# kaushikcfd/feinsum

Measured on AMD Instinct MI355X. Metric: GFLOP/s on DG-wave p=4 grad einsum (1e6 elems per GPU, fp64); fraction of roofline in `roofline`, higher is better.
Workload: dtype f64

## Files before the change

### feinsum_amd/_hip.py

```python

from __future__ import annotations

import ctypes as C
import os
from pathlib import Path
from typing import Optional, Sequence, Tuple

import numpy as np

from feinsum_amd.diagnostics import HipLibraryError, InvalidParameterError

FE_OK, FE_EINVAL, FE_EUNSUPPORTED, FE_EHIP = 0, -1, -2, -3
VARIANT_AUTO, VARIANT_GENERIC, VARIANT_MFMA, VARIANT_TILED, VARIANT_MFMA_SPLIT = 0, 1, 2, 3, 4
VARIANTS = {"auto": VARIANT_AUTO, "generic": VARIANT_GENERIC, "mfma": VARIANT_MFMA, "tiled": VARIANT_TILED,
            "mfma_split": VARIANT_MFMA_SPLIT}

FAMILY_F32 = 0x100
FAMILY_ACC = 0x200
FAMILY_FIELDS_F32 = 0x400


class ArgPack(C.Structure):

    _fields_ = [
# ... 79 lines not shown
    "fe_launch": (_int, [_i32, C.POINTER(ArgPack), _p]),
    "fe_grad3d_mixed_f64": (_int, [_p, _p, _pp, _pp, _i64, _i32, _i32, _i32, _p]),
    "fe_div3d_mixed_f64": (_int, [_p, _p, _pp, _pp, _i64, _i32, _i32, _i32, _p]),
    "fe_facemass_mixed_f64": (_int, [_p, _p, _pp, _pp, _i64, _i32, _i32, _i32, _i32, _i32, _p]),
    "fe_grad3d_strided_f64": (_int, [_p, _i64, _p, _pp, _pp, _i64, _i64, _i32, _i32, _i32, _p]),
    "fe_div3d_strided_f64": (_int, [_p, _i64, _p, _pp, _i64, _pp, _i64, _i32, _i32, _i32, _p]),
    "fe_facemass_strided_f64": (_int, [_p, _i64, _p, _pp, _i64, _pp, _i64, _i32, _i32, _i32, _i32, _i32, _p]),
    "fe_launch_f32": (_int, [_i32, C.POINTER(ArgPack), _p]),
    "fe_set_tail_rounds": (_int, [_i32]),
    "fe_set_tail_min_rounds": (_int, [_i32]),
    "fe_stream_retired": (_int, [_p]),
    "fe_tail_check": (_int, [_i32, C.POINTER(_i64), C.POINTER(_i32), C.POINTER(_i32), C.POINTER(_i32)]),
    "fe_capture_id": (_int, [_p, C.POINTER(C.c_uint64)]),
    "fe_graph_retired": (_int, [C.c_uint64]),
    "fe_tail_stats": (_int, [C.POINTER(_i64), _i32]),
    "fe_tail_plant": (_int, [_p, C.c_uint32]),
    "fe_set_temporal_loads_mib": (_int, [_i32]),
    "fe_set_write_through_mib": (_int, [_i32]),
    "fe_last_launch_info": (_int, [C.POINTER(_i64), _i32]),
    "fe_set_div_interleave": (_i64, [_i64]),
    "fe_set_div_quarter_tail": (_int, [_i32]),
    "fe_set_grad_quarter_tail": (_int, [_i32]),
    "fe_set_grad_staggered_start": (_int, [_i32]),
    "fe_set_phase_priority_p5": (_int, [_i32]),
    "fe_set_cu_limit": (_int, [_i32]),
    "fe_time_launches": (_int, [_i32, C.POINTER(ArgPack), _i32, _p, C.POINTER(C.c_float)]),
    "fe_einsum_generic": (_int, [C.POINTER(EinsumDesc), _pp, _p, _p]),
    "fe_einsum_contract": (_int, [C.POINTER(EinsumDesc), _pp, _p, _p]),
    "fe_einsum_contract_groups": (_int, [C.POINTER(EinsumDesc), C.POINTER(_i32), C.POINTER(_i32)]),
    "fe_einsum_reduce_plan": (_int, [C.POINTER(EinsumDesc), C.POINTER(_i32), C.POINTER(_i64), C.POINTER(_size)]),
    "fe_einsum_reduce": (_int, [C.POINTER(EinsumDesc), _pp, _p, _p, _size, _p]),
    "fe_geomadj_f64": (_int, [_p, _p, _p, _p, _i64, _i32, _i32, _i32, _i32, _i64, _i64, _i64, _p]),
    "fe_facemass_adj_f64": (_int, [_p, _p, _pp, _pp, _pp, _p, _i64, _i32, _i32, _i32, _i32, _i32, _p]),
    "fe_opgrad_plan": (_int, [_i64, _i32, C.POINTER(_i64), C.POINTER(_size)]),
    "fe_opgrad_f64": (_int, [_p, _pp, _pp, _p, _i64, _i32, _i32, _i32, _i32, _i64, _i64, _i64, _i64, _i64, _i64, _p, _size,
                          _p]),
    "fe_facemass_opgrad_f64": (_int, [_p, _pp, _pp, _p, _i64, _i32, _i32, _i32, _i32, _i32, _p, _size, _p]),
}
EXPORTED_SYMBOLS = tuple(SIGNATURES)


def library_path() -> Path:
    env = os.environ.get("FEINSUM_HIP_LIB")
    return Path(env) if env else Path(__file__).resolve().parent / "libfeinsum_hip.so"


# ... 432 lines not shown
    d["mixed_fields"] = bool(d["kind"] & 32)
    d["plain_field_loads"] = bool(d["kind"] & 64)
    d["element_slice"] = bool(d["kind"] & 128)
    d["kind"] = "B build interleaved" if d["kind"] & 4 else "default"
    return d


def set_phase_priority_p5(on: bool) -> bool:
    return bool(load_library().fe_set_phase_priority_p5(1 if on else 0))


def set_div_quarter_tail(on: bool) -> bool:
    return bool(load_library().fe_set_div_quarter_tail(1 if on else 0))


def set_grad_quarter_tail(on: bool) -> bool:
    return bool(load_library().fe_set_grad_quarter_tail(int(on)))


def set_grad_staggered_start(on: bool) -> bool:
    return bool(load_library().fe_set_grad_staggered_start(1 if on else 0))


def set_div_interleave(tiles: int) -> int:
    return int(load_library().fe_set_div_interleave(int(tiles)))


def set_write_through_mib(mib: int) -> int:
    return int(load_library().fe_set_write_through_mib(int(mib)))


def set_temporal_loads_mib(mib: int) -> int:
    return int(load_library().fe_set_temporal_loads_mib(int(mib)))
```

### feinsum_amd/csrc/fe_common.h

```cpp
#pragma once
#include <hip/hip_runtime.h>
#include <stdint.h>

namespace fe {

typedef double v4d __attribute__((ext_vector_type(4)));
typedef double v2d __attribute__((ext_vector_type(2)));

#define FE_AS1 __attribute__((address_space(1)))
#define FE_AS3 __attribute__((address_space(3)))

constexpr int kMaxFields = 8;
struct FieldPtrs {
    const double* v[kMaxFields];
    double* out[kMaxFields];
};

__device__ __forceinline__ const double* field_in(const FieldPtrs& P, int k) {
    const double* p = P.v[0];
#pragma unroll
    for (int q = 1; q < kMaxFields; ++q) p = (k == q) ? P.v[q] : p;
    return p;
}
__device__ __forceinline__ double* field_out(const FieldPtrs& P, int k) {
// ... 236 lines not shown

__device__ __forceinline__ void balance_priority(bool younger_half, int iteration) {
    if (younger_half) {
        if (iteration & 1) __builtin_amdgcn_s_setprio(1);
        else __builtin_amdgcn_s_setprio(0);
    }
}

template <class F>
__device__ __forceinline__ void remainder_items(int64_t e_begin, int64_t E, int Np, unsigned bid, unsigned nblk,
                                                F item) {
    const int64_t n = (E - e_begin) * Np;
    if (n <= 0) return;
    const unsigned per = blockDim.x;
    const int64_t want = (n + per - 1) / per;
    const unsigned k = want < (int64_t)nblk ? (unsigned)want : nblk;
    const unsigned half = (nblk + 1) / 2;
    const unsigned first = half >= k ? half - k : 0;
    if (bid < first || bid >= first + k) return;
    for (int64_t idx = (int64_t)(bid - first) * per + threadIdx.x; idx < n; idx += (int64_t)k * per)
        item(e_begin + idx / Np, (int)(idx % Np));
}

}
```

### feinsum_amd/csrc/fe_grad.h

```cpp
#pragma once
#include <type_traits>

#include "fe_common.h"
#include "fe_generic.h"

namespace fe {

constexpr int grad_row_tiles(int np) {
    int t = 1;
    while (4 * ((4 * t) / 3) < np) ++t;
    return t;
}

template <int NP, int M>
struct GradGeom {
    static constexpr int TEL = 16 * M;
    static constexpr int RT = grad_row_tiles(NP);
    static constexpr int TG = (4 * RT) / 3;
    static constexpr int KS = (NP + 3) / 4;
    static constexpr int TILE_D = TEL * NP;
    static constexpr int SUB_D = 16 * NP;
    static constexpr int U_CHUNKS = TILE_D / 2;
    static constexpr int U_INSTR = (U_CHUNKS + 63) / 64;
    static constexpr int J_ROW_CHUNKS = TEL / 2;
    static constexpr int J_CHUNKS = 9 * J_ROW_CHUNKS;
    static constexpr int J_INSTR = (J_CHUNKS + 63) / 64;
    static constexpr int SUB_CHUNKS = SUB_D / 2;
    static constexpr int SUB_INSTR = (SUB_CHUNKS + 63) / 64;
    static constexpr int LOADS = U_INSTR + J_INSTR;
    static constexpr int PLANE_STORES = M * SUB_INSTR;
    static constexpr int STORES = 3 * PLANE_STORES;
    static constexpr int ACC_LOADS = STORES;
    struct WaveLds {
        double u[2][TILE_D];
        double j[2][9 * TEL];
    };
    struct WaveOut {
        double o[2][SUB_D];
    };
    static constexpr int WAVES = 4;
    static constexpr int OP_D = 3 * NP * NP;
    static constexpr int IN_BYTES = (int)sizeof(WaveLds) * WAVES;
    static constexpr int OUT_BYTES = (int)sizeof(WaveOut) * WAVES;
    static constexpr int OP_BYTES = (OP_D * 8 + 15) / 16 * 16;
    static constexpr int LDS_BYTES = IN_BYTES + (OUT_BYTES > OP_BYTES ? OUT_BYTES : OP_BYTES);
    static_assert(4 * TG >= NP, "row permutation must cover every i");
    static_assert(LOADS + STORES + ACC_LOADS <= 60, "counted vmcnt must fit the 6-bit field");
    static_assert(2 * LDS_BYTES <= 160 * 1024, "two blocks per CU");
};

struct GradFields {
    const double* j[3];
    const double* u[kMaxFields];
    double* out[kMaxFields][3];
};

__device__ __forceinline__ const double* grad_field_u(const GradFields& P, int k) {
    const double* p = P.u[0];
#pragma unroll
    for (int q = 1; q < kMaxFields; ++q) p = (k == q) ? P.u[q] : p;
    return p;
}
__device__ __forceinline__ double* grad_plane_out(const GradFields& P, int k, int x) {
    double* p = P.out[0][x];
#pragma unroll
    for (int q = 1; q < kMaxFields; ++q) p = (k == q) ? P.out[q][x] : p;
    return p;
}
// ... 20 lines not shown
            J[(int64_t)(x * 3 + 2) * E + e] * t2;
}

__device__ __forceinline__ void grad3d_item_ld(const double* __restrict__ J, const double* __restrict__ D,
                                               const double* __restrict__ u, double* __restrict__ out, int64_t ldJ,
                                               int64_t ldOut, int Np, int64_t e, int i, int opT) {
    double t0 = 0.0, t1 = 0.0, t2 = 0.0;
    const double* ue = u + e * Np;
    const int si = opT ? 1 : Np, sj = opT ? Np : 1;
    const double* d0 = D + (int64_t)0 * Np * Np + (int64_t)i * si;
    const double* d1 = D + (int64_t)1 * Np * Np + (int64_t)i * si;
    const double* d2 = D + (int64_t)2 * Np * Np + (int64_t)i * si;
#pragma unroll 5
    for (int j = 0; j < Np; ++j) {
        const double uj = ue[j];
        t0 += d0[j * sj] * uj;
        t1 += d1[j * sj] * uj;
        t2 += d2[j * sj] * uj;
    }
    for (int x = 0; x < 3; ++x)
        out[((int64_t)x * ldOut + e) * Np + i] =
            J[(int64_t)(x * 3 + 0) * ldJ + e] * t0 + J[(int64_t)(x * 3 + 1) * ldJ + e] * t1 +
            J[(int64_t)(x * 3 + 2) * ldJ + e] * t2;
}

__global__ __launch_bounds__(256) void grad3d_generic_ld_kernel(
    const double* __restrict__ J, const double* __restrict__ D, const double* __restrict__ u,
    double* __restrict__ out, int64_t E, int64_t ldJ, int64_t ldOut, int Np, int opT) {
    const int64_t idx = (int64_t)blockIdx.x * 256 + threadIdx.x;
    if (idx >= E * Np) return;
    grad3d_item_ld(J, D, u, out, ldJ, ldOut, Np, idx / Np, (int)(idx % Np), opT);
}

__device__ __forceinline__ void grad3d_item_acc(const double* __restrict__ J, const double* __restrict__ D,
                                                const double* __restrict__ u, double* __restrict__ out, int64_t E,
                                                int Np, int64_t e, int i, int opT, double alpha, double beta) {
    double t0 = 0.0, t1 = 0.0, t2 = 0.0;
    const double* ue = u + e * Np;
    const int si = opT ? 1 : Np, sj = opT ? Np : 1;
    const double* d0 = D + (int64_t)0 * Np * Np + (int64_t)i * si;
    const double* d1 = D + (int64_t)1 * Np * Np + (int64_t)i * si;
    const double* d2 = D + (int64_t)2 * Np * Np + (int64_t)i * si;
#pragma unroll 5
    for (int j = 0; j < Np; ++j) {
        const double uj = ue[j];
        t0 += d0[j * sj] * uj;
// ... 88 lines not shown
            fe::fe_dbg_tile[GLOBAL_WAVE][LANE] = reinterpret_cast<unsigned long long*>(LDS_END)[(WAVE) * 16 + (LANE)];   \
    } while (0)
#else
#define FE_TILE_STAMP(ENABLED, LDS_END, WAVE, LANE, IT, K) do {} while (0)
#define FE_TILE_STAMPS_OUT(ENABLED, LDS_END, WAVE, LANE, GLOBAL_WAVE) do {} while (0)
#endif

template <int N>
struct GradOldValues {
    v2d v[2][N];
};
template <>
struct GradOldValues<0> {};
template <int NP, int N>
__device__ __forceinline__ void grad_load_old(const double* op, int lane, v2d (&dst)[N]) {
    constexpr int CHUNKS = 16 * NP / 2;
#pragma unroll
    for (int c = 0; c < N; ++c) {
        const int qc = c * 64 + lane;
        if ((c + 1) * 64 <= CHUNKS || qc < CHUNKS) dst[c] = __builtin_nontemporal_load(reinterpret_cast<const v2d*>(op + 2 * qc));
    }
}

template <int NP, int M, int kDbg = 0, bool kPlain = true, bool kPrep = false, bool kDyn = false, bool kAcc = false, bool kLd = false>
__device__ __forceinline__ void grad3d_mfma_body(
    const GradFields& P, const double* __restrict__ D, const void* __restrict__ prep, int nb, int nx_, int64_t E,
    int64_t nTiles, int op_flags, const unsigned bid, const unsigned nblk, unsigned* __restrict__ tail = nullptr,
    int64_t t_static = 0, const double alpha = 1.0, const double beta = 0.0, const int64_t ldJ = 0, const int64_t ldOut = 0) {
    static_assert(!kDyn || (kPlain && !kPrep), "dynamic walk: plain launches of one field");
    static_assert(!kLd || (kPlain && !kPrep && !kAcc && kDbg == 0), "element slices: plain grad, the plain operator");
    static_assert(!kAcc || (kPlain && !kPrep && !kDyn && kDbg == 0), "accumulating launches: plain grad, static walk, the plain operator");
    constexpr bool kAccAhead = kAcc && NP != 35;
    const bool acc_reads = kAcc && beta != 0.0;
    const int opT = op_flags & 1;
    const bool tload = (op_flags & kOpLoadsTemporal) != 0;
    const bool wthrough = kPlain && !kAcc && (op_flags & kOpStoresWriteThrough) != 0;
    const int nx = kPlain ? 3 : nx_;
    using G = GradGeom<NP, M>;
    using WaveLds = typename G::WaveLds;
    extern __shared__ __attribute__((aligned(16))) char smem[];
#ifdef FE_EXPERIMENTS
    const unsigned long long t_entry = (kDbg & 32) ? __builtin_amdgcn_s_memrealtime() : 0;
#endif
    if constexpr (kPlain && !kPrep && !kDyn && M == 1 && !kAcc && !kLd) {
        if ((op_flags & kOpStaggeredStart) && ((bid >> 3) & 1))
            for (int i = 0; i < kStaggerSleeps; ++i) __builtin_amdgcn_s_sleep(16);
    }
    const int lane = threadIdx.x & 63;
    const int wave = __builtin_amdgcn_readfirstlane(threadIdx.x >> 6);
    WaveLds* L = reinterpret_cast<WaveLds*>(smem) + wave;
    typename G::WaveOut* LO = reinterpret_cast<typename G::WaveOut*>(smem + G::IN_BYTES) + wave;
    const int n = lane & 15, g = lane >> 4;
#ifdef FE_EXPERIMENTS
    constexpr bool x_no_mfma = (kDbg & 1) != 0, x_no_stores = (kDbg & 2) != 0, x_plain_stores = (kDbg & 4) != 0, x_no_loads = (kDbg & 8) != 0,
// ... 37 lines not shown
        else grad_issue_j<NP, M, kPlain>(P, E, phys(tile), lane, lds_addr_uniform(L->j[0]));
        if (nb > 1) {
            grad_issue_u<NP, M, kNT>(P.u[1], phys(tile), lane, lds_addr_uniform(L->u[1]), tload);
            pre = true;
            return 1;
        }
        return 3;
    };
    auto remainder = [&](const double* Dsrc) {
        remainder_items(nTiles * G::TEL, E, NP, bid, nblk, [&](int64_t e, int i) {
            for (int k = 0; k < nb; ++k) {
                const double* uk = grad_field_u(P, k);
                if (kPlain) {
                    if constexpr (kLd) grad3d_item_ld(P.j[0], Dsrc, uk, grad_plane_out(P, k, 0), ldJ, ldOut, NP, e, i, opT);
                    else if constexpr (kAcc) grad3d_item_acc(P.j[0], Dsrc, uk, grad_plane_out(P, k, 0), E, NP, e, i, opT, alpha, beta);
                    else grad3d_item(P.j[0], Dsrc, uk, grad_plane_out(P, k, 0), E, NP, e, i, opT);
                } else {
                    double* const o[3] = {grad_plane_out(P, k, 0), grad_plane_out(P, k, 1), grad_plane_out(P, k, 2)};
#pragma unroll
                    for (int x = 0; x < 3; ++x)
                        if (o[x]) divcomp3d_item(P.j[x], Dsrc, uk, o[x], E, NP, e, i, opT, 0);
                }
            }
        });
    };
    int dbg_it = 0;
#ifdef FE_EXPERIMENTS
    if ((kDbg & 32) && lane < 16) reinterpret_cast<unsigned long long*>(smem + G::LDS_BYTES)[wave * 16 + lane] = 0;
#endif
    auto compute_unit = [&](int64_t tile_, int fk, const double* ut, const double* jt, auto with_acc) {
        constexpr bool kHaveAcc = decltype(with_acc)::value;
        FE_TILE_STAMP(x_stamps, smem + G::LDS_BYTES, wave, lane, dbg_it, 0);
        double* out_x[3];
        out_x[0] = grad_plane_out(P, fk, 0);
        if constexpr (kLd) out_x[1] = out_x[0] + ldOut * NP;
        else out_x[1] = kPlain ? out_x[0] + E * NP : grad_plane_out(P, fk, 1);
        if constexpr (kLd) out_x[2] = out_x[0] + 2 * ldOut * NP;
        else out_x[2] = kPlain ? out_x[0] + 2 * E * NP : grad_plane_out(P, fk, 2);
        int obuf = 0;
        const int64_t e0 = phys(tile_) * G::TEL;
        GradOldValues<kAcc ? G::SUB_INSTR : 0> old;
        if constexpr (kAccAhead) {
            if (acc_reads) grad_load_old<NP>(out_x[0] + e0 * NP, lane, old.v[0]);
        }
#pragma unroll
        for (int m = 0; m < M; ++m) {
// ... 258 lines not shown
        fk = nk;
        tile = nt;
        ub ^= 1;
        if (next_new_tile) jbuf ^= 1;
    };
    auto first_top = [&]() {
        if constexpr (kDyn) {
            if (use_dyn) {
                dyn_init();
                dyn_top();
                return;
            }
        }
        static_top();
    };

    if constexpr (kPrep) {
        load_prepared_fragments<G::RT * G::KS>(prep, lane, [&](int f, double v) { afrag[f / G::KS][f % G::KS] = v; });
        issue_first_units();
        prepared_fragments_landed();
        remainder(D);
    } else {
        stage_operator_dma<G::OP_D>(D, lds_addr_uniform(smem + G::IN_BYTES), wave, lane);
        const int units_issued = issue_first_units();
        switch (units_issued) {
            case 1: wait_vmcnt<G::LOADS + G::U_INSTR>(); break;
            case 3: wait_vmcnt<G::LOADS>(); break;
            default: wait_vmcnt<0>(); break;
        }
#ifdef FE_EXPERIMENTS
        if ((kDbg & 32) && lane == 0 && bid * G::WAVES + wave < 4096) fe_dbg_phase[bid * G::WAVES + wave][0] = __builtin_amdgcn_s_memrealtime();
#endif
        __syncthreads();
#ifdef FE_EXPERIMENTS
        if ((kDbg & 32) && lane == 0 && bid * G::WAVES + wave < 4096) fe_dbg_phase[bid * G::WAVES + wave][1] = __builtin_amdgcn_s_memrealtime();
#endif

        const double* dl = reinterpret_cast<const double*>(smem + G::IN_BYTES);
        remainder(dl);
        const int gp = n & 3, q = n >> 2;
        const int istride = opT ? 1 : NP, jstride = opT ? NP : 1;
        if constexpr (kFusedFirst) {
            static_assert(4 * (G::RT - 1) <= 3 * G::TG && 3 * G::TG + (4 * (G::RT - 1) - 1) / 3 < NP && 4 * G::KS - 5 < NP,
                          "padding rows in the last row tile only, padding columns in the last k-step only");
            const double* rowp[G::RT];
            bool rowok_last = true;
#pragma unroll
            for (int t = 0; t < G::RT; ++t) {
                const int s_ = 4 * t + q;
                const int r = s_ % 3, i = G::TG * gp + s_ / 3;
                if (t == G::RT - 1) rowok_last = (s_ < 3 * G::TG) && (i < NP);
                rowp[t] = dl + r * (NP * NP) + (i < NP ? i : 0) * istride + g * jstride;
            }
            const bool jok_last = 4 * (G::KS - 1) + g < NP;
            static_assert(4 * G::KS - NP <= 1 && (G::OP_D + NP + 1) * 8 <= G::LDS_BYTES - G::IN_BYTES, "the padding column stays inside the staging area");
            const int kstep = 4 * jstride;
            auto read_step = [&](int ks) {
#pragma unroll
                for (int t = 0; t < G::RT; ++t) afrag[t][ks] = rowp[t][ks * kstep];
            };
            auto fix_step = [&](int ks) {
#pragma unroll
// ... 147 lines not shown
            }
            wave_lds_fence();
        }
    }
    if constexpr (kDyn) {
        if (reportedb) {
            const unsigned pool_blocks = (nblk / (8 * kTailPools)) * 8 + (unsigned)max(0, min(8, (int)(nblk % (8 * kTailPools)) - 8 * pool));
            const unsigned before = tail_wait<G::STORES, 1>();
            if (before + 1 == pool_blocks * G::WAVES && lane == 0) {
                __hip_atomic_store(counter, 0u, __ATOMIC_RELAXED, __HIP_MEMORY_SCOPE_AGENT);
                __hip_atomic_store(done, 0u, __ATOMIC_RELAXED, __HIP_MEMORY_SCOPE_AGENT);
            }
        }
    }
#ifdef FE_EXPERIMENTS
    write_stamps(iteration);
#endif
}

template <int NP, int M, int kDbg = 0, bool kPlain = true, bool kPrep = false>
__global__ __launch_bounds__(256, 2) void grad3d_mfma_kernel(
    GradFields P, const double* __restrict__ D, const void* __restrict__ prep, int nb, int nx, int64_t E,
    int64_t nTiles, int opT) {
    grad3d_mfma_body<NP, M, kDbg, kPlain, kPrep>(P, D, prep, nb, nx, E, nTiles, opT, blockIdx.x, gridDim.x);
}

template <int NP, int M>
__global__ __launch_bounds__(256, 2) void grad3d_mfma_acc_kernel(
    GradFields P, const double* __restrict__ D, int64_t E, int64_t nTiles, int opT, double alpha, double beta) {
    grad3d_mfma_body<NP, M, 0, true, false, false, true>(P, D, nullptr, 1, 3, E, nTiles, opT, blockIdx.x, gridDim.x, nullptr, 0,
                                                         alpha, beta);
}

template <int NP, int M>
__global__ __launch_bounds__(256, 2) void grad3d_mfma_strided_kernel(
    GradFields P, const double* __restrict__ D, int nb, int64_t E, int64_t ldJ, int64_t ldOut, int64_t nTiles, int opT) {
    grad3d_mfma_body<NP, M, 0, true, false, false, false, true>(P, D, nullptr, nb, 3, E, nTiles, opT, blockIdx.x, gridDim.x, nullptr, 0,
                                                                1.0, 0.0, ldJ, ldOut);
}

template <int NP, int M>
__global__ __launch_bounds__(256, 2) FE_TAIL_KERNEL_ATTR void grad3d_mfma_strided_tail_kernel(
    GradFields P, const double* __restrict__ D, int nb, int64_t E, int64_t ldJ, int64_t ldOut, int64_t nTiles, int opT,
    unsigned* __restrict__ tail, int64_t t_static) {
    grad3d_mfma_body<NP, M, 0, true, false, true, false, true>(P, D, nullptr, nb, 3, E, nTiles, opT, blockIdx.x, gridDim.x, tail, t_static,
                                                               1.0, 0.0, ldJ, ldOut);
}
// ... 26 lines not shown
```

### feinsum_amd/csrc/feinsum_hip.hip

```cpp
#include <hip/hip_runtime.h>

#include <cmath>
#include <cstdarg>
#include <cstdio>
#include <cstdlib>
#include <cstring>
#include <algorithm>
#include <atomic>
#include <mutex>
#include <string>
#include <tuple>
#include <type_traits>
#include <unordered_map>
#include <utility>
#include <vector>

#include "../../include/feinsum_hip.h"
#include "fe_common.h"
#include "fe_adjoint.h"
#include "fe_opgrad.h"
#include "fe_contract.h"
#include "fe_div.h"
#include "fe_einsum.h"
#include "fe_reduce.h"
// ... 276 lines not shown
int write_through_flag(int64_t output_bytes) {
    return output_bytes <= g_write_through_output_bytes.load(std::memory_order_relaxed) ? fe::kOpStoresWriteThrough : 0;
}

constexpr long long kDivInterleaveTiles = 37500;
std::atomic<long long> g_div_interleave_tiles{[] { const char* e = getenv("FEINSUM_DIV_INTERLEAVE_TILES"); return e ? atoll(e) : kDivInterleaveTiles; }()};

std::atomic<int> g_div_quarter_tail{[] { const char* e = getenv("FEINSUM_DIV_QUARTER_TAIL"); return e ? atoi(e) : 1; }()};

constexpr int kGradQuarterDen = 8;
std::atomic<int> g_grad_quarter_tail{[] { const char* e = getenv("FEINSUM_GRAD_QUARTER_TAIL"); return e ? atoi(e) : 1; }()};
int grad_quarter_flag(int m, int nb, int64_t nTiles, int64_t waves) {
    const int64_t ragged = nTiles % waves;
    const int setting = g_grad_quarter_tail.load(std::memory_order_relaxed);
    const int64_t den = setting >= 4 ? setting : kGradQuarterDen;
    return (m == 1 && nb == 1 && setting != 0 && nTiles > waves && ragged > 0 && den * ragged <= waves) ? fe::kOpQuarterTail : 0;
}

std::atomic<int> g_grad_staggered_start{[] { const char* e = getenv("FEINSUM_GRAD_STAGGERED_START"); return e ? atoi(e) : 1; }()};
int grad_stagger_flag(int np, int m, int nb, int64_t nTiles, int64_t waves) {
    return (np == 35 && m == 1 && nb == 1 && g_grad_staggered_start.load(std::memory_order_relaxed) && 2 * nTiles >= 5 * waves) ? fe::kOpStaggeredStart : 0;
}

std::atomic<int> g_phase_priority_p5{[] { const char* e = getenv("FEINSUM_PHASE_PRIORITY_P5"); return e ? atoi(e) : 0; }()};
int phase_priority_flag_p5() { return g_phase_priority_p5.load(std::memory_order_relaxed) ? fe::kOpPhasePriority : 0; }

struct LastLaunch {
    int valid = 0, dynamic_walk = 0, temporal_loads = 0, write_through = 0, blocks = 0, waves_per_block = 0, kind = 0, bodies = 0;
    long long tiles = 0, static_tiles = 0;
};
thread_local LastLaunch g_last_launch;
void forget_last_launch() { g_last_launch.valid = 0; }
void note_launch(bool dynamic, int flags, unsigned blocks, int waves_per_block, int64_t tiles, int64_t static_tiles, int kind = 0, int bodies = 1) {
    LastLaunch& L = g_last_launch;
    L.valid = 1;
    L.dynamic_walk = dynamic ? 1 : 0;
    L.temporal_loads = (flags & fe::kOpLoadsTemporal) ? 1 : 0;
    L.write_through = (flags & fe::kOpStoresWriteThrough) ? 1 : 0;
    L.blocks = (int)blocks;
    L.waves_per_block = waves_per_block;
    L.kind = kind;
    L.bodies = bodies;
    L.tiles = tiles;
    L.static_tiles = dynamic ? static_tiles : tiles;
}

unsigned grid_for(int64_t nTiles, int wavesPerBlock, int per_cu) {
    const int64_t blocks = (nTiles + wavesPerBlock - 1) / wavesPerBlock;
    const int64_t cap = per_cu * (int64_t)device_cu_count();
    return (unsigned)(blocks < cap ? blocks : cap);
}
unsigned persistent_grid(int64_t nTiles, int wavesPerBlock) { return grid_for(nTiles, wavesPerBlock, 8 / wavesPerBlock); }


template <auto K>
int configured(const char* what, int lds_bytes, int threads, int blocks_per_cu) {
    static PerDeviceOnce once;
    return once.run([&] { return configure_kernel(K, what, lds_bytes, threads, blocks_per_cu); });
}

struct Geometry {
    int waves, threads, lds, resident, per_cu;
};

struct Walk {
    int64_t tiles[3];
    int bodies;
    unsigned tickets;
    bool units;
};
Walk walk_static(int64_t tiles) { return {{tiles, 0, 0}, 1, 0u, false}; }
Walk walk_tickets(int64_t tiles, bool tickets = true, bool units = false) { return {{tiles, 0, 0}, 1, tickets ? 1u : 0u, units}; }

struct Launch {
    unsigned grid;
    int waves_per_block;
    int64_t t_static[3];
    unsigned* tail;
    int64_t waves() const { return (int64_t)grid * waves_per_block; }
};

template <typename... A>
struct Call {
    int flags, kind;
    std::tuple<A...> args;
};
template <typename... A>
Call<A...> call(int flags, int kind, A... args) { return {flags, kind, std::tuple<A...>(args...)}; }

template <auto K, auto KT = nullptr, typename SC, typename TC = std::nullptr_t>
int mfma_launch(hipStream_t s, const Walk& w, const Geometry& g, const char* what, SC static_call, const char* tail_what = nullptr,
                TC tail_call = nullptr) {
    if (int rc = configured<K>(what, g.lds, g.threads, g.resident)) return rc;
    int64_t most = 0, tiles = 0, t_static = 0;
    for (int b = 0; b < w.bodies; ++b) {
        most = w.tiles[b] > most ? w.tiles[b] : most;
        tiles += w.tiles[b];
    }
    Launch L = {grid_for(most, g.waves, g.per_cu), g.waves, {w.tiles[0], w.tiles[1], w.tiles[2]}, nullptr};
    bool dynamic = false;
    if constexpr (KT != nullptr) {
        for (int b = 0; b < w.bodies; ++b)
            if (w.tickets & (1u << b)) {
                L.t_static[b] = tail_static_tiles(w.tiles[b], L.grid, g.waves, w.bodies > 1, w.units);
                dynamic = dynamic || L.t_static[b] < w.tiles[b];
            }
        if (dynamic) L.tail = tail_slot(s, w.bodies);
    }
    for (int b = 0; b < w.bodies; ++b) t_static += L.t_static[b];
    auto enqueue = [&](auto kernel, const auto& c) {
        std::apply([&](auto... a) { hipLaunchKernelGGL(kernel, dim3(L.grid), dim3(g.threads), g.lds, s, a...); }, c.args);
        note_launch(L.tail != nullptr, c.flags, L.grid, g.waves, tiles, t_static, c.kind, w.bodies);
        return FE_OK;
    };
    if constexpr (KT != nullptr) {
        if (L.tail) {
            if (int rc = configured<KT>(tail_what, g.lds, g.threads, g.resident)) return rc;
            return enqueue(KT, tail_call(L));
        }
    }
    return enqueue(K, static_call(L));
}
// ... 128 lines not shown
    const Geometry dbg_geo = {G::WAVES, 256, G::LDS_BYTES, 1, 8 / G::WAVES},
                   stamps_geo = {G::WAVES, 256, G::LDS_BYTES + fe::kDbgTileLdsBytes, 1, 8 / G::WAVES};
#define FE_GRAD_CASE(DBG, GEO) \
    case DBG: return mfma_launch<fe::grad3d_mfma_kernel<NP, M, DBG>>(s, walk_static(nTiles), GEO, "experiment", args);
    switch (NP == 35 ? dbg : 0) {
        FE_GRAD_CASE(1, dbg_geo)
        FE_GRAD_CASE(2, dbg_geo)
        FE_GRAD_CASE(3, dbg_geo)
        FE_GRAD_CASE(4, dbg_geo)
        FE_GRAD_CASE(8, dbg_geo)
        FE_GRAD_CASE(9, dbg_geo)
        FE_GRAD_CASE(10, dbg_geo)
        FE_GRAD_CASE(11, dbg_geo)
        FE_GRAD_CASE(16, dbg_geo)
        FE_GRAD_CASE(20, dbg_geo)
        case 32:
            if (gsec)
                return mfma_launch<fe::grad3d_mfma_kernel<NP, M, 32, true, true>>(
                    s, walk_static(nTiles), stamps_geo, "experiment",
                    [&](const Launch&) { return call(opT, 0, P, D, gsec, nb, nx, E, nTiles, opT); });
            return mfma_launch<fe::grad3d_mfma_kernel<NP, M, 32>, fe::grad3d_mfma_tail_kernel<NP, M, 32>>(
                s, walk_tickets(nTiles, nb == 1), stamps_geo, "experiment",
                [&](const Launch& L) {
                    const int f = opT | (nb == 1 ? write_through_flag(3 * (int64_t)NP * E * 8) | grad_quarter_flag(M, nb, nTiles, L.waves()) : 0);
                    return call(f, 0, P, D, nullptr, nb, nx, E, nTiles, f);
                },
                "experiment", tail_args);
        FE_GRAD_CASE(64, dbg_geo)
        FE_GRAD_CASE(96, stamps_geo)
        FE_GRAD_CASE(128, dbg_geo)
        default: break;
    }
#undef FE_GRAD_CASE
#else
    (void)dbg;
#endif
    if (gsec) {
        snprintf(what, sizeof(what), "grad Np=%d M=%d, prepared operator", NP, M);
        return mfma_launch<fe::grad3d_mfma_kernel<NP, M, 0, true, true>>(
            s, walk_static(nTiles), geo, what, [&](const Launch&) { return call(opT, 0, P, D, gsec, nb, nx, E, nTiles, opT); });
    }
    auto static_args = [&](const Launch& L) {
        const int f = opT | (nb == 1 ? write_through_flag(3 * (int64_t)NP * E * 8) | grad_quarter_flag(M, nb, nTiles, L.waves()) |
                                           grad_stagger_flag(NP, M, nb, nTiles, L.waves())
                                     : 0);
        return call(f, ((f & fe::kOpQuarterTail) ? 8 : 0) | ((f & fe::kOpStaggeredStart) ? 16 : 0), P, D, nullptr, nb, nx, E, nTiles, f);
    };
    snprintf(what, sizeof(what), "grad Np=%d M=%d", NP, M);
    if (nb == 1) {
        snprintf(tail_what, sizeof(tail_what), "grad Np=%d M=%d, dynamic walk", NP, M);
        const int f = opT | write_through_flag(3 * (int64_t)NP * E * 8);
        return mfma_launch<fe::grad3d_mfma_kernel<NP, M, 0>, fe::grad3d_mfma_tail_kernel<NP, M>>(
            s, walk_tickets(nTiles), geo, what, static_args, tail_what,
            [&](const Launch& L) { return call(f, 0, P, D, nb, E, nTiles, f, L.tail, L.t_static[0]); });
    }
    snprintf(tail_what, sizeof(tail_what), "grad Np=%d M=%d x b, dynamic walk", NP, M);
    return mfma_launch<fe::grad3d_mfma_kernel<NP, M, 0>, fe::grad3d_mfma_tail_kernel<NP, M, 0, true>>(
        s, walk_tickets(nTiles), geo, what, static_args, tail_what, tail_args);
}

template <int NP, int M>
int launch_div(const double* J, const double* D, const void* prep, const fe::FieldPtrs& P, int nb, int64_t E, int dbg,
               int opT, hipStream_t s, int64_t* e_done) {
    using G = fe::DivGeom<NP, M>;
    const int64_t nTiles = E / G::TEL;
    *e_done = nTiles > 0 ? E : 0;
    if (nTiles == 0) return FE_OK;
    opT |= temporal_flag((9 + 3 * (int64_t)nb * NP) * E * 8, kTemporalFloorDiv, kTemporalCapDivMib);
    const Geometry geo = {G::WAVES, 256, G::LDS_BYTES, G::BLOCKS_PER_CU, 8 / G::WAVES};
    char what[64], tail_what[64];
    auto args = [&](const Launch&) { return call(opT & ~fe::kOpStoresWriteThrough, 0, J, D, nullptr, P, nb, E, nTiles, opT, 0); };
    auto tail_args = [&](const Launch& L) { return call(opT, 0, J, D, P, nb, E, nTiles, opT, L.tail, L.t_static[0]); };
#ifdef FE_EXPERIMENTS
    const Geometry dbg_geo = {G::WAVES, 256, G::LDS_BYTES, 1, 8 / G::WAVES},
                   stamps_geo = {G::WAVES, 256, G::LDS_BYTES + fe::kDbgTileLdsBytes, 1, 8 / G::WAVES};
#define FE_DIV_CASE(DBG) \
// ... 2261 lines not shown
}

int fe_set_write_through_mib(int32_t mib) {
    return (int)(g_write_through_output_bytes.exchange(mib < 0 ? 0 : (long long)mib << 20) >> 20);
}

int fe_last_launch_info(int64_t* out, int32_t n) {
    if (!out || n < 1) return fail(FE_EINVAL, "fe_last_launch_info: bad arguments");
    const LastLaunch& L = g_last_launch;
    const int64_t v[FE_LAST_LAUNCH_INFO] = {L.valid, L.dynamic_walk, L.temporal_loads, L.write_through, L.blocks, L.waves_per_block, L.kind, L.bodies,
                                            L.tiles, L.static_tiles};
    for (int k = 0; k < n && k < FE_LAST_LAUNCH_INFO; ++k) out[k] = v[k];
    return n < FE_LAST_LAUNCH_INFO ? n : FE_LAST_LAUNCH_INFO;
}

int fe_set_div_quarter_tail(int32_t on) {
    return g_div_quarter_tail.exchange(on ? 1 : 0);
}

int fe_set_grad_quarter_tail(int32_t on) {
    return g_grad_quarter_tail.exchange(on < 0 ? 0 : (on == 2 || on == 3) ? 1 : on);
}

int fe_set_grad_staggered_start(int32_t on) {
    return g_grad_staggered_start.exchange(on ? 1 : 0);
}

int fe_set_tail_min_rounds(int32_t rounds) {
    return g_tail_min_rounds_v.exchange(rounds < 2 ? 2 : rounds);
}

int64_t fe_set_div_interleave(int64_t tiles) {
    return g_div_interleave_tiles.exchange(tiles < 0 ? 0 : tiles);
}

int fe_set_phase_priority_p5(int32_t on) {
    return g_phase_priority_p5.exchange(on ? 1 : 0);
}

int fe_set_cu_limit(int32_t cus) {
    return g_cu_limit.exchange(cus < 0 ? 0 : cus);
}

int fe_stream_retired(void* stream) {
    int dev = 0;
    FE_HIP_CHECK(hipGetDevice(&dev));
// ... 696 lines not shown
```

### include/feinsum_hip.h

```cpp
#ifndef FEINSUM_HIP_H
#define FEINSUM_HIP_H

#include <stddef.h>
#include <stdint.h>

#ifdef __cplusplus
extern "C" {
#endif

#define FE_OK            0
#define FE_EINVAL       -1
#define FE_EUNSUPPORTED -2
#define FE_EHIP         -3

#define FE_VARIANT_AUTO    0
#define FE_VARIANT_GENERIC 1
#define FE_VARIANT_MFMA    2
#define FE_VARIANT_TILED   3
#define FE_VARIANT_MFMA_SPLIT 4

#define FE_FAMILY_GRAD     1
#define FE_FAMILY_DIV      2
#define FE_FAMILY_GRADDIV  3
#define FE_FAMILY_FACEMASS 4
// ... 182 lines not shown

int fe_set_tail_rounds(int32_t rounds);
int fe_set_tail_min_rounds(int32_t rounds);

int fe_stream_retired(void* stream);
int fe_tail_check(int32_t repair, int64_t* dirty_words, int32_t* groups, int32_t* streams, int32_t* captured);
#define FE_TAIL_STATS 12
int fe_capture_id(void* stream, uint64_t* id);
int fe_graph_retired(uint64_t capture_id);
int fe_tail_stats(int64_t* out, int32_t n);
int fe_tail_plant(void* stream, uint32_t value);

int fe_set_temporal_loads_mib(int32_t mib);

int fe_set_write_through_mib(int32_t mib);

#define FE_LAST_LAUNCH_INFO 10
int fe_last_launch_info(int64_t* out, int32_t n);

int64_t fe_set_div_interleave(int64_t tiles);
int fe_set_div_quarter_tail(int32_t on);
int fe_set_grad_quarter_tail(int32_t on);
int fe_set_grad_staggered_start(int32_t on);
int fe_set_phase_priority_p5(int32_t on);

int fe_set_cu_limit(int32_t cus);

int fe_time_launches(int32_t family, const fe_argpack* args, int32_t n_launches,
                     void* stream, float* ms_out);

#define FE_MAX_EINSUM_OPERANDS 8
#define FE_MAX_EINSUM_INDICES  8
#define FE_DTYPE_F64 0
#define FE_DTYPE_F32 1
#define FE_DTYPE_OPERAND_F32(p) (1 << (8 + (p)))
#define FE_DTYPE_OPERAND_F32_MASK (((1 << FE_MAX_EINSUM_OPERANDS) - 1) << 8)

typedef struct fe_einsum_desc {
    int32_t n_operands, n_out, n_sum, dtype;
    int64_t out_extent[FE_MAX_EINSUM_INDICES];
    int64_t sum_extent[FE_MAX_EINSUM_INDICES];
    int64_t op_out_stride[FE_MAX_EINSUM_OPERANDS][FE_MAX_EINSUM_INDICES];
    int64_t op_sum_stride[FE_MAX_EINSUM_OPERANDS][FE_MAX_EINSUM_INDICES];
} fe_einsum_desc;

typedef struct fe_einsum_ptrs {
// ... 44 lines not shown
```

Measured before the change: 42060.

## Prefetch grad remainder elements into LDS via DMA and add spare remainder blocks

Result: no change. 42070 (median of 2 runs) (+0.0%).

```diff
diff --git a/feinsum_amd/_hip.py b/feinsum_amd/_hip.py
--- a/feinsum_amd/_hip.py
+++ b/feinsum_amd/_hip.py
@@ -125,6 +125,7 @@
     "fe_set_div_quarter_tail": (_int, [_i32]),
     "fe_set_grad_quarter_tail": (_int, [_i32]),
     "fe_set_grad_staggered_start": (_int, [_i32]),
+    "fe_set_remainder_prefetch": (_int, [_i32]),
     "fe_set_phase_priority_p5": (_int, [_i32]),
     "fe_set_cu_limit": (_int, [_i32]),
     "fe_time_launches": (_int, [_i32, C.POINTER(ArgPack), _i32, _p, C.POINTER(C.c_float)]),
@@ -603,6 +604,10 @@
     return bool(load_library().fe_set_grad_staggered_start(1 if on else 0))
 
 
+def set_remainder_prefetch(on: bool) -> bool:
+    return bool(load_library().fe_set_remainder_prefetch(1 if on else 0))
+
+
 def set_div_interleave(tiles: int) -> int:
     return int(load_library().fe_set_div_interleave(int(tiles)))
 
diff --git a/feinsum_amd/csrc/fe_common.h b/feinsum_amd/csrc/fe_common.h
--- a/feinsum_amd/csrc/fe_common.h
+++ b/feinsum_amd/csrc/fe_common.h
@@ -282,4 +282,47 @@
         item(e_begin + idx / Np, (int)(idx % Np));
 }
 
-}
+constexpr int kOpRemainderPrefetch = 512;
+struct RemainderBlocks {
+    unsigned first, k;
+};
+__device__ __forceinline__ RemainderBlocks remainder_blocks(int64_t n, unsigned per, unsigned nblk, unsigned tile_blocks, bool staggered) {
+    if (n <= 0) return {0u, 0u};
+    const int64_t want = (n + per - 1) / per;
+    if (nblk > tile_blocks) {
+        const unsigned spare = nblk - tile_blocks;
+        const unsigned k = want < (int64_t)spare ? (unsigned)want : spare;
+        return {nblk - k, k};
+    }
+    const unsigned k = want < (int64_t)nblk ? (unsigned)want : nblk;
+    const unsigned half = (nblk + 1) / 2;
+    unsigned first = half >= k ? half - k : 0;
+    if (staggered && k <= 8 && half >= 16) {
+        unsigned group = (half - 1) >> 3;
+        if (group & 1) --group;
+        first = group * 8 + 8 - k;
+    }
+    return {first, k};
+}
+template <class F>
+__device__ __forceinline__ void remainder_items_on(RemainderBlocks rb, int64_t e_begin, int64_t E, int Np, unsigned bid, F item) {
+    if (bid < rb.first || bid >= rb.first + rb.k) return;
+    const int64_t n = (E - e_begin) * Np;
+    const unsigned per = blockDim.x;
+    for (int64_t idx = (int64_t)(bid - rb.first) * per + threadIdx.x; idx < n; idx += (int64_t)rb.k * per)
+        item(e_begin + idx / Np, (int)(idx % Np));
+}
+template <int MAXD>
+__device__ __forceinline__ void remainder_copy_dma(const double* __restrict__ g, int doubles, unsigned lds, int wave, int lane) {
+    constexpr int kInstr = (MAXD / 2 + 255) / 256;
+    const char* gb = reinterpret_cast<const char*>(g);
+    const int chunks = doubles >> 1;
+#pragma unroll
+    for (int c = 0; c < kInstr; ++c) {
+        const int q0 = (c * 4 + wave) * 64;
+        if (q0 + lane < chunks) glds16(gb + (int64_t)(q0 + lane) * 16, lds + q0 * 16);
+    }
+    if ((doubles & 1) && wave == 0 && lane < 2) glds4(gb + (int64_t)(doubles - 1) * 8 + lane * 4, lds + (doubles - 1) * 8);
+}
+
+}
diff --git a/feinsum_amd/csrc/fe_grad.h b/feinsum_amd/csrc/fe_grad.h
--- a/feinsum_amd/csrc/fe_grad.h
+++ b/feinsum_amd/csrc/fe_grad.h
@@ -43,7 +43,16 @@
     static constexpr int IN_BYTES = (int)sizeof(WaveLds) * WAVES;
     static constexpr int OUT_BYTES = (int)sizeof(WaveOut) * WAVES;
     static constexpr int OP_BYTES = (OP_D * 8 + 15) / 16 * 16;
-    static constexpr int LDS_BYTES = IN_BYTES + (OUT_BYTES > OP_BYTES ? OUT_BYTES : OP_BYTES);
+    static constexpr int REM_MAX = TEL - 1;
+    static constexpr int REM_U_BYTES = (REM_MAX * NP * 8 + 15) / 16 * 16;
+    static constexpr int REM_J_BYTES = (9 * REM_MAX * 8 + 15) / 16 * 16;
+    static constexpr int REM_JT_BYTES = 80;
+    static constexpr int REM_OFF = IN_BYTES + OP_BYTES;
+    static constexpr int REM_END = REM_OFF + REM_U_BYTES + REM_J_BYTES + REM_JT_BYTES;
+    static constexpr int STAGE_BYTES = OUT_BYTES > OP_BYTES ? OUT_BYTES : OP_BYTES;
+    static constexpr int LDS_BYTES = IN_BYTES + STAGE_BYTES > REM_END ? IN_BYTES + STAGE_BYTES : REM_END;
+    static_assert(REM_OFF % 16 == 0 && REM_U_BYTES % 16 == 0 && REM_J_BYTES % 16 == 0, "LDS-DMA destinations are 16-byte aligned");
+    static_assert(NP != 35 || REM_END <= IN_BYTES + OUT_BYTES, "p = 4: the remainder's operands fit the output region behind the operator");
     static_assert(4 * TG >= NP, "row permutation must cover every i");
     static_assert(LOADS + STORES + ACC_LOADS <= 60, "counted vmcnt must fit the 6-bit field");
     static_assert(2 * LDS_BYTES <= 160 * 1024, "two blocks per CU");
@@ -110,6 +119,25 @@
         out[((int64_t)x * ldOut + e) * Np + i] =
             J[(int64_t)(x * 3 + 0) * ldJ + e] * t0 + J[(int64_t)(x * 3 + 1) * ldJ + e] * t1 +
             J[(int64_t)(x * 3 + 2) * ldJ + e] * t2;
+}
+
+__device__ __forceinline__ void grad3d_item_lds(const double* jp, int js, const double* D, const double* ue,
+                                                double* __restrict__ out, int64_t E, int Np, int64_t e, int i, int opT) {
+    double t0 = 0.0, t1 = 0.0, t2 = 0.0;
+    const int si = opT ? 1 : Np, sj = opT ? Np : 1;
+    const double* d0 = D + (int64_t)0 * Np * Np + (int64_t)i * si;
+    const double* d1 = D + (int64_t)1 * Np * Np + (int64_t)i * si;
+    const double* d2 = D + (int64_t)2 * Np * Np + (int64_t)i * si;
+#pragma unroll 5
+    for (int j = 0; j < Np; ++j) {
+        const double uj = ue[j];
+        t0 += d0[j * sj] * uj;
+        t1 += d1[j * sj] * uj;
+        t2 += d2[j * sj] * uj;
+    }
+    for (int x = 0; x < 3; ++x)
+        out[((int64_t)x * E + e) * Np + i] =
+            jp[(x * 3 + 0) * js] * t0 + jp[(x * 3 + 1) * js] * t1 + jp[(x * 3 + 2) * js] * t2;
 }
 
 __global__ __launch_bounds__(256) void grad3d_generic_ld_kernel(
@@ -244,7 +272,8 @@
     }
 }
 
-template <int NP, int M, int kDbg = 0, bool kPlain = true, bool kPrep = false, bool kDyn = false, bool kAcc = false, bool kLd = false>
+template <int NP, int M, int kDbg = 0, bool kPlain = true, bool kPrep = false, bool kDyn = false, bool kAcc = false, bool kLd = false,
+          bool kRem = false>
 __device__ __forceinline__ void grad3d_mfma_body(
     const GradFields& P, const double* __restrict__ D, const void* __restrict__ prep, int nb, int nx_, int64_t E,
     int64_t nTiles, int op_flags, const unsigned bid, const unsigned nblk, unsigned* __restrict__ tail = nullptr,
@@ -252,6 +281,7 @@
     static_assert(!kDyn || (kPlain && !kPrep), "dynamic walk: plain launches of one field");
     static_assert(!kLd || (kPlain && !kPrep && !kAcc && kDbg == 0), "element slices: plain grad, the plain operator");
     static_assert(!kAcc || (kPlain && !kPrep && !kDyn && kDbg == 0), "accumulating launches: plain grad, static walk, the plain operator");
+    static_assert(!kRem || (kPlain && !kPrep && !kDyn && !kAcc && !kLd), "prefetched remainder: plain grad, static walk, the plain operator");
     constexpr bool kAccAhead = kAcc && NP != 35;
     const bool acc_reads = kAcc && beta != 0.0;
     const int opT = op_flags & 1;
@@ -335,6 +365,46 @@
                         if (o[x]) divcomp3d_item(P.j[x], Dsrc, uk, o[x], E, NP, e, i, opT, 0);
                 }
             }
+        });
+    };
+    const int64_t rem_e0 = nTiles * G::TEL;
+    const int rem = (int)(E - rem_e0);
+    const int rem_even = rem & ~1;
+    RemainderBlocks rem_blocks = {0u, 0u};
+    bool rem_on = false, rem_mine = false;
+    if constexpr (kRem) {
+        rem_on = (op_flags & kOpRemainderPrefetch) != 0 && nb == 1 && rem > 0;
+        if (rem_on) {
+            rem_blocks = remainder_blocks((int64_t)rem * NP, 256u, nblk, (unsigned)((nTiles + G::WAVES - 1) / G::WAVES),
+                                          (op_flags & kOpStaggeredStart) != 0);
+            rem_mine = bid >= rem_blocks.first && bid < rem_blocks.first + rem_blocks.k;
+        }
+    }
+    auto issue_remainder_copy = [&]() {
+        const unsigned base = lds_addr_uniform(smem + G::REM_OFF);
+        remainder_copy_dma<G::REM_MAX * NP>(P.u[0] + rem_e0 * NP, rem * NP, base, wave, lane);
+        const int rc = rem >> 1, chunks = 9 * rc;
+        constexpr int kInstr = (9 * (G::REM_MAX / 2) + 255) / 256;
+#pragma unroll
+        for (int c = 0; c < kInstr; ++c) {
+            const int q0 = (c * 4 + wave) * 64, q = q0 + lane;
+            if (q < chunks) {
+                const int row = q / rc, col = q - row * rc;
+                glds16(reinterpret_cast<const char*>(P.j[0] + (int64_t)row * E + rem_e0) + col * 16, base + G::REM_U_BYTES + q0 * 16);
+            }
+        }
+        if ((rem & 1) && wave == 0 && lane < 18)
+            glds4(reinterpret_cast<const char*>(P.j[0] + (int64_t)(lane >> 1) * E + rem_e0 + (rem - 1)) + (lane & 1) * 4,
+                  base + G::REM_U_BYTES + G::REM_J_BYTES);
+    };
+    auto remainder_lds = [&](const double* Dsrc) {
+        const double* ru = reinterpret_cast<const double*>(smem + G::REM_OFF);
+        const double* rj = reinterpret_cast<const double*>(smem + G::REM_OFF + G::REM_U_BYTES);
+        const double* rjt = reinterpret_cast<const double*>(smem + G::REM_OFF + G::REM_U_BYTES + G::REM_J_BYTES);
+        remainder_items_on(rem_blocks, rem_e0, E, NP, bid, [&](int64_t e, int i) {
+            const int el = (int)(e - rem_e0);
+            const bool even_part = el < rem_even;
+            grad3d_item_lds(even_part ? rj + el : rjt, even_part ? rem_even : 1, Dsrc, ru + el * NP, grad_plane_out(P, 0, 0), E, NP, e, i, opT);
         });
     };
     int dbg_it = 0;
@@ -639,6 +709,9 @@
         remainder(D);
     } else {
         stage_operator_dma<G::OP_D>(D, lds_addr_uniform(smem + G::IN_BYTES), wave, lane);
+        if constexpr (kRem) {
+            if (rem_mine) issue_remainder_copy();
+        }
         const int units_issued = issue_first_units();
         switch (units_issued) {
             case 1: wait_vmcnt<G::LOADS + G::U_INSTR>(); break;
@@ -654,7 +727,12 @@
 #endif
 
         const double* dl = reinterpret_cast<const double*>(smem + G::IN_BYTES);
-        remainder(dl);
+        if constexpr (kRem) {
+            if (rem_on) remainder_lds(dl);
+            else remainder(dl);
+        } else {
+            remainder(dl);
+        }
         const int gp = n & 3, q = n >> 2;
         const int istride = opT ? 1 : NP, jstride = opT ? NP : 1;
         if constexpr (kFusedFirst) {
@@ -848,7 +926,7 @@
 __global__ __launch_bounds__(256, 2) void grad3d_mfma_kernel(
     GradFields P, const double* __restrict__ D, const void* __restrict__ prep, int nb, int nx, int64_t E,
     int64_t nTiles, int opT) {
-    grad3d_mfma_body<NP, M, kDbg, kPlain, kPrep>(P, D, prep, nb, nx, E, nTiles, opT, blockIdx.x, gridDim.x);
+    grad3d_mfma_body<NP, M, kDbg, kPlain, kPrep, false, false, false, kPlain && !kPrep>(P, D, prep, nb, nx, E, nTiles, opT, blockIdx.x, gridDim.x);
 }
 
 template <int NP, int M>
diff --git a/feinsum_amd/csrc/feinsum_hip.hip b/feinsum_amd/csrc/feinsum_hip.hip
--- a/feinsum_amd/csrc/feinsum_hip.hip
+++ b/feinsum_amd/csrc/feinsum_hip.hip
@@ -322,6 +322,12 @@
     return (np == 35 && m == 1 && nb == 1 && g_grad_staggered_start.load(std::memory_order_relaxed) && 2 * nTiles >= 5 * waves) ? fe::kOpStaggeredStart : 0;
 }
 
+std::atomic<int> g_remainder_prefetch{[] { const char* e = getenv("FEINSUM_REMAINDER_PREFETCH"); return e ? atoi(e) : 1; }()};
+int remainder_prefetch_flag(int nb) { return (nb == 1 && g_remainder_prefetch.load(std::memory_order_relaxed)) ? fe::kOpRemainderPrefetch : 0; }
+int remainder_spare_blocks(int flag, int64_t rem_elements, int np) {
+    return flag ? (int)((rem_elements * np + 255) / 256) : 0;
+}
+
 std::atomic<int> g_phase_priority_p5{[] { const char* e = getenv("FEINSUM_PHASE_PRIORITY_P5"); return e ? atoi(e) : 0; }()};
 int phase_priority_flag_p5() { return g_phase_priority_p5.load(std::memory_order_relaxed) ? fe::kOpPhasePriority : 0; }
 
@@ -368,6 +374,7 @@
     int bodies;
     unsigned tickets;
     bool units;
+    int spare = 0;
 };
 Walk walk_static(int64_t tiles) { return {{tiles, 0, 0}, 1, 0u, false}; }
 Walk walk_tickets(int64_t tiles, bool tickets = true, bool units = false) { return {{tiles, 0, 0}, 1, tickets ? 1u : 0u, units}; }
@@ -398,6 +405,10 @@
         tiles += w.tiles[b];
     }
     Launch L = {grid_for(most, g.waves, g.per_cu), g.waves, {w.tiles[0], w.tiles[1], w.tiles[2]}, nullptr};
+    if (w.spare > 0) {
+        const int64_t cap = g.per_cu * (int64_t)device_cu_count(), with_spare = (int64_t)L.grid + w.spare;
+        if ((int64_t)L.grid < cap) L.grid = (unsigned)(with_spare < cap ? with_spare : cap);
+    }
     bool dynamic = false;
     if constexpr (KT != nullptr) {
         for (int b = 0; b < w.bodies; ++b)
@@ -572,7 +583,9 @@
             return mfma_launch<fe::grad3d_mfma_kernel<NP, M, 32>, fe::grad3d_mfma_tail_kernel<NP, M, 32>>(
                 s, walk_tickets(nTiles, nb == 1), stamps_geo, "experiment",
                 [&](const Launch& L) {
-                    const int f = opT | (nb == 1 ? write_through_flag(3 * (int64_t)NP * E * 8) | grad_quarter_flag(M, nb, nTiles, L.waves()) : 0);
+                    const int f = opT | (nb == 1 ? write_through_flag(3 * (int64_t)NP * E * 8) | grad_quarter_flag(M, nb, nTiles, L.waves()) |
+                                                       grad_stagger_flag(NP, M, nb, nTiles, L.waves()) | remainder_prefetch_flag(nb)
+                                                 : 0);
                     return call(f, 0, P, D, nullptr, nb, nx, E, nTiles, f);
                 },
                 "experiment", tail_args);
@@ -592,7 +605,7 @@
     }
     auto static_args = [&](const Launch& L) {
         const int f = opT | (nb == 1 ? write_through_flag(3 * (int64_t)NP * E * 8) | grad_quarter_flag(M, nb, nTiles, L.waves()) |
-                                           grad_stagger_flag(NP, M, nb, nTiles, L.waves())
+                                           grad_stagger_flag(NP, M, nb, nTiles, L.waves()) | remainder_prefetch_flag(nb)
                                      : 0);
         return call(f, ((f & fe::kOpQuarterTail) ? 8 : 0) | ((f & fe::kOpStaggeredStart) ? 16 : 0), P, D, nullptr, nb, nx, E, nTiles, f);
     };
@@ -600,8 +613,10 @@
     if (nb == 1) {
         snprintf(tail_what, sizeof(tail_what), "grad Np=%d M=%d, dynamic walk", NP, M);
         const int f = opT | write_through_flag(3 * (int64_t)NP * E * 8);
+        Walk w = walk_tickets(nTiles);
+        w.spare = remainder_spare_blocks(remainder_prefetch_flag(nb), E - nTiles * G::TEL, NP);
         return mfma_launch<fe::grad3d_mfma_kernel<NP, M, 0>, fe::grad3d_mfma_tail_kernel<NP, M>>(
-            s, walk_tickets(nTiles), geo, what, static_args, tail_what,
+            s, w, geo, what, static_args, tail_what,
             [&](const Launch& L) { return call(f, 0, P, D, nb, E, nTiles, f, L.tail, L.t_static[0]); });
     }
     snprintf(tail_what, sizeof(tail_what), "grad Np=%d M=%d x b, dynamic walk", NP, M);
@@ -2909,6 +2924,10 @@
     return g_grad_quarter_tail.exchange(on < 0 ? 0 : (on == 2 || on == 3) ? 1 : on);
 }
 
+int fe_set_remainder_prefetch(int32_t on) {
+    return g_remainder_prefetch.exchange(on ? 1 : 0);
+}
+
 int fe_set_grad_staggered_start(int32_t on) {
     return g_grad_staggered_start.exchange(on ? 1 : 0);
 }
diff --git a/include/feinsum_hip.h b/include/feinsum_hip.h
--- a/include/feinsum_hip.h
+++ b/include/feinsum_hip.h
@@ -228,6 +228,7 @@
 int fe_set_div_quarter_tail(int32_t on);
 int fe_set_grad_quarter_tail(int32_t on);
 int fe_set_grad_staggered_start(int32_t on);
+int fe_set_remainder_prefetch(int32_t on);
 int fe_set_phase_priority_p5(int32_t on);
 
 int fe_set_cu_limit(int32_t cus);
```
